# mengcaopku/DCNet

Hardware: AMD Instinct MI355X
Metric: clips/sec (T=8, 416x416, bs8) fwd+bwd (higher is better)
Workload: dtype f32; 1 GPU; T=8 416x416 bs8/GPU L=20 fp32, 64 img/GPU/step as pairs, fwd+5 losses+bwd+RMSprop; arith=f16x2-split MFMA, fp32 accumulate, parallelism=dp1, ranks_seen=1, reducer=none, step=hipGraph replay (fwd+losses+bwd+RMSprop), sampler=mt

## Files before the change

dcnet_amd/csrc/conv1.hip:

```cpp
#include "igemm.h"
#include "prof.h"

namespace {

typedef _Float16 f16x8_t __attribute__((ext_vector_type(8)));
typedef _Float16 f16x4_t __attribute__((ext_vector_type(4)));
typedef __attribute__((address_space(3))) void lds_void;

constexpr unsigned C1_OOB = 0x80000000u;

__device__ __forceinline__ float c1_pow2_scale(unsigned amax_bits) {
  const int be = (int)((amax_bits >> 23) & 0xFF);
  if (be == 0 || be == 255) return 1.f;
  int e = 14 - (be - 126);
  e = e > 100 ? 100 : (e < -100 ? -100 : e);
  return __uint_as_float((unsigned)(e + 127) << 23);
}

#ifndef C1_OCC
#define C1_OCC 4
#endif
template <int SA, int SB, int NI, int MI>
__global__ __launch_bounds__(256, (NI == 4 && MI == 1) ? C1_OCC : 2) void conv1_kernel(const IgemmParams p) {
  constexpr int BM = 128 * MI, BN = 32 * NI;
  constexpr int ASTAGE = BM * 64, BPLANE = BN * 32, BSTAGE = 2 * BPLANE;
  constexpr int AP = 4 * MI;
  constexpr int NLD = AP > NI ? AP : NI;
  extern __shared__ __attribute__((aligned(1024))) unsigned char smem1[];
  const int tid = threadIdx.x, lane = tid & 63;
  const int wave = __builtin_amdgcn_readfirstlane(tid >> 6);
  const int gn = p.Co / BN;
  const int lin = xcd_remap(blockIdx.x, gridDim.x);
  const int bm = lin / gn, bn = lin - bm * gn;
  const int M = p.M, m0 = bm * BM;
  const int cpt = p.Ci >> 4;
  const int kiters = p.ntaps * cpt;
  const int hsws = p.Hs * p.Ws;
  const bool plain = p.ntaps == 1 && p.dense_out && p.isy == 1 && p.isx == 1 && p.tap_dy[0] == 0 && p.tap_dx[0] == 0 &&
                     p.Ws == p.Wi && p.Hs == p.Hi;

  const float sa = c1_pow2_scale(amax_read(p.amax_a)), sb = p.b_scale[0];

  const int n0 = m0 / hsws;
  const long long img = (long long)p.Hi * p.Wi * p.ldi;
  const float* a_base = p.in + (long long)n0 * img;
  const long long a_bytes = ((long long)(p.N - n0) * img - p.ldi + p.Ci) * 4;
  const __amdgpu_buffer_rsrc_t a_rs = __builtin_amdgcn_make_buffer_rsrc((void*)a_base, 0, a_bytes > 0x7FFFFFF0LL ? 0x7FFFFFF0 : (int)a_bytes, 0x00020000);
  const __amdgpu_buffer_rsrc_t b_rs = __builtin_amdgcn_make_buffer_rsrc((void*)p.wt, 0, (int)((long long)p.Co * p.ldw * 4), 0x00020000);

  const bool loads_a = wave < 2;
  unsigned voff[NLD], msk[NLD];
#pragma unroll
  for (int e = 0; e < NLD; ++e) { voff[e] = C1_OOB; msk[e] = 0; }
  if (loads_a) {
#pragma unroll
    for (int e = 0; e < AP; ++e) {
      const int j = AP * (wave & 1) + e;
      const int row = 16 * j + (lane >> 2), cp = lane & 3, c = cp ^ ((row >> 2) & 3);
      const int m = m0 + row;
      if (m < M) {
        if (plain) { voff[e] = (unsigned)((m - n0 * hsws) * p.ldi * 4 + c * 16); msk[e] = 1u; }
        else {
          const int n = m / hsws, rem = m - n * hsws;
          const int i = rem / p.Ws, jx = rem - i * p.Ws;
          const int iy0 = i * p.isy, ix0 = jx * p.isx;
          voff[e] = (unsigned)((((n - n0) * p.Hi + iy0) * p.Wi + ix0) * p.ldi * 4 + c * 16);
          unsigned mk = 0;
          for (int t = 0; t < p.ntaps; ++t)
            if ((unsigned)(iy0 + p.tap_dy[t]) < (unsigned)p.Hi && (unsigned)(ix0 + p.tap_dx[t]) < (unsigned)p.Wi) mk |= 1u << t;
          msk[e] = mk;
        }
      }
    }
  } else {
#pragma unroll
    for (int e = 0; e < NI; ++e) {
      const int plane = wave & 1, rr = 32 * e + (lane >> 1), kh = (lane & 1) ^ ((rr >> 3) & 1);
      voff[e] = (unsigned)((bn * BN + rr) * p.ldw * 4 + (2 * kh + plane) * 16);
      msk[e] = 0xFFFFu;
    }
  }
  const __amdgpu_buffer_rsrc_t my_rs = loads_a ? a_rs : b_rs;
  const int my_dst = loads_a ? AP * (wave & 1) * 1024 : SA * ASTAGE + (wave & 1) * BPLANE;
  const int my_n = loads_a ? AP : NI;

  int k_tap = 0, k_c = 0, k_done = 0;
  auto issue = [&]() {
    const bool live = k_done < kiters;
    const unsigned bit = 1u << k_tap;
    int delta = 0; unsigned soff = 0;
    if (live) {
      if (loads_a) { delta = (p.tap_dy[k_tap] * p.Wi + p.tap_dx[k_tap]) * p.ldi * 4; soff = (unsigned)k_c * 64u; }
      else soff = (unsigned)(p.tap_w[k_tap] + k_c * 16) * 4u;
    }
    unsigned char* st = smem1 + (loads_a ? (k_done % SA) * ASTAGE : (k_done % SB) * BSTAGE) + my_dst;
#pragma unroll
    for (int e = 0; e < NLD; ++e)
      if (e < my_n)
        __builtin_amdgcn_raw_ptr_buffer_load_lds(my_rs, (lds_void*)(st + e * 1024), 16,
                                                 (int)((live && (msk[e] & bit)) ? voff[e] + (unsigned)delta : C1_OOB), (int)soff, 0, 0);
    ++k_done; ++k_c;
    if (k_c == cpt) { k_c = 0; ++k_tap; }
  };

  const int kh = lane >> 5;
  int a_rd0[MI], a_rd1[MI];
#pragma unroll
  for (int mi = 0; mi < MI; ++mi) {
    const int ar = (wave * MI + mi) * 32 + (lane & 31);
    a_rd0[mi] = ar * 64 + (((2 * kh) ^ ((ar >> 2) & 3)) << 4);
    a_rd1[mi] = ar * 64 + (((2 * kh + 1) ^ ((ar >> 2) & 3)) << 4);
  }
  int b_rd[NI];
#pragma unroll
  for (int ni = 0; ni < NI; ++ni) {
    const int row = ni * 32 + (lane & 31);
    b_rd[ni] = SA * ASTAGE + row * 32 + (((kh ^ (row >> 3)) & 1) << 4);
  }

  f32x16 acc[MI][NI];
#pragma unroll
  for (int mi = 0; mi < MI; ++mi)
#pragma unroll
    for (int ni = 0; ni < NI; ++ni)
#pragma unroll
      for (int r = 0; r < 16; ++r) acc[mi][ni][r] = 0.f;

  for (int s = 0; s < (loads_a ? SA : SB) - 1; ++s) issue();

  for (int it = 0; it < kiters; ++it) {
    if (loads_a) asm volatile("s_waitcnt vmcnt(%0)" :: "n"((SA - 2) * AP) : "memory");
    else asm volatile("s_waitcnt vmcnt(%0)" :: "n"((SB - 2) * NI) : "memory");
    __builtin_amdgcn_s_barrier();
    asm volatile("" ::: "memory");
    issue();
    const unsigned char* st = smem1 + (it % SA) * ASTAGE;
    const unsigned char* sb_ = smem1 + (it % SB) * BSTAGE;
    f16x8_t bh[NI], bl[NI];
#pragma unroll
    for (int ni = 0; ni < NI; ++ni) {
      bh[ni] = *reinterpret_cast<const f16x8_t*>(sb_ + b_rd[ni]);
      bl[ni] = *reinterpret_cast<const f16x8_t*>(sb_ + BPLANE + b_rd[ni]);
    }
    f16x8_t ah[MI], al[MI];
#pragma unroll
    for (int mi = 0; mi < MI; ++mi) {
      const f32x4 x0 = *reinterpret_cast<const f32x4*>(st + a_rd0[mi]), x1 = *reinterpret_cast<const f32x4*>(st + a_rd1[mi]);
      const f32x4 t0 = x0 * sa, t1 = x1 * sa;
#pragma unroll
      for (int e = 0; e < 4; ++e) { ah[mi][e] = (_Float16)t0[e]; ah[mi][4 + e] = (_Float16)t1[e]; }
#pragma unroll
      for (int e = 0; e < 4; ++e) { al[mi][e] = (_Float16)(t0[e] - (float)ah[mi][e]); al[mi][4 + e] = (_Float16)(t1[e] - (float)ah[mi][4 + e]); }
    }
#pragma unroll
    for (int mi = 0; mi < MI; ++mi)
#pragma unroll
      for (int ni = 0; ni < NI; ++ni) acc[mi][ni] = __builtin_amdgcn_mfma_f32_32x32x16_f16(al[mi], bh[ni], acc[mi][ni], 0, 0, 0);
#pragma unroll
    for (int mi = 0; mi < MI; ++mi)
#pragma unroll
      for (int ni = 0; ni < NI; ++ni) acc[mi][ni] = __builtin_amdgcn_mfma_f32_32x32x16_f16(ah[mi], bl[ni], acc[mi][ni], 0, 0, 0);
#pragma unroll
    for (int mi = 0; mi < MI; ++mi)
#pragma unroll
      for (int ni = 0; ni < NI; ++ni) acc[mi][ni] = __builtin_amdgcn_mfma_f32_32x32x16_f16(ah[mi], bh[ni], acc[mi][ni], 0, 0, 0);
  }
  asm volatile("s_waitcnt vmcnt(0)" ::: "memory");
  __syncthreads();

  const float dq = 1.f / (sa * sb);
#pragma unroll
  for (int mi = 0; mi < MI; ++mi)
#pragma unroll
    for (int ni = 0; ni < NI; ++ni) acc[mi][ni] *= dq;

  float* __restrict__ gout = p.out;
  auto out_pix = [&](int m) -> size_t {
    if (p.dense_out) return (size_t)m;
    const int n = m / hsws, rem = m - n * hsws;
    const int i = rem / p.Ws, jx = rem - i * p.Ws;
    return ((size_t)n * p.Ho + p.oy0 + i * p.osy) * p.Wo + p.ox0 + jx * p.osx;
  };
  if (p.accumulate) {
#pragma unroll
    for (int mi = 0; mi < MI; ++mi)
#pragma unroll
      for (int r = 0; r < 16; ++r) {
        const int m = m0 + (wave * MI + mi) * 32 + 4 * kh + (r & 3) + 8 * (r >> 2);
        if (m >= M) continue;
        const size_t pix = out_pix(m);
#pragma unroll
        for (int ni = 0; ni < NI; ++ni) acc[mi][ni][r] += gout[pix * p.ldo + bn * BN + ni * 32 + (lane & 31)];
      }
  }
  if (p.stats) {
    float* red = reinterpret_cast<float*>(smem1);
#pragma unroll
    for (int ni = 0; ni < NI; ++ni) {
      float s = 0.f, ss = 0.f;
      if (p.bt_y) {
        const int co = bn * BN + ni * 32 + (lane & 31);
        const float mu = p.bt_mean[co], is = p.bt_invstd[co], ga = p.bt_gamma ? p.bt_gamma[co] : 1.f, be = p.bt_beta ? p.bt_beta[co] : 0.f;
        const float* yb = p.bt_y + co;
        float yv[MI][16];
#pragma unroll
        for (int mi = 0; mi < MI; ++mi)
#pragma unroll
          for (int r = 0; r < 16; ++r) {
            const int m = m0 + (wave * MI + mi) * 32 + 4 * kh + (r & 3) + 8 * (r >> 2);
            yv[mi][r] = yb[(size_t)(m < M ? m : M - 1) * p.Co];
          }
#pragma unroll
        for (int mi = 0; mi < MI; ++mi)
#pragma unroll
          for (int r = 0; r < 16; ++r) {
            const int m = m0 + (wave * MI + mi) * 32 + 4 * kh + (r & 3) + 8 * (r >> 2);
            const float xh = (yv[mi][r] - mu) * is;
            float g = acc[mi][ni][r];
            if (p.bt_act == DCN_ACT_LEAKY) g = (ga * xh + be <= 0.f) ? g * p.bt_slope : g;
            g = m < M ? g : 0.f;
            s += g; ss += g * xh;
          }
      } else {
#pragma unroll
        for (int mi = 0; mi < MI; ++mi)
#pragma unroll
          for (int r = 0; r < 16; ++r) { const float v = acc[mi][ni][r]; s += v; ss = __builtin_fmaf(v, v, ss); }
      }
      s += __shfl_xor(s, 32); ss += __shfl_xor(ss, 32);
      if (lane < 32) {
        red[(0 * 4 + wave) * BN + ni * 32 + lane] = s;
        red[(1 * 4 + wave) * BN + ni * 32 + lane] = ss;
      }
    }
    __syncthreads();
    for (int idx = tid; idx < 2 * BN; idx += 256) {
      const int which = idx / BN, col = idx - which * BN;
      float t = 0.f;
#pragma unroll
      for (int w = 0; w < 4; ++w) t += red[(which * 4 + w) * BN + col];
      p.stats[((size_t)bm * 2 + which) * p.Co + bn * BN + col] = t;
    }
  }
  float sc[NI], sh[NI];
#pragma unroll
  for (int ni = 0; ni < NI; ++ni) {
    const int co = bn * BN + ni * 32 + (lane & 31);
    sc[ni] = p.scale ? p.scale[co] : 1.f;
    sh[ni] = p.shift ? p.shift[co] : 0.f;
  }
  float vmax = 0.f;
#pragma unroll
  for (int mi = 0; mi < MI; ++mi)
#pragma unroll
    for (int r = 0; r < 16; ++r) {
      const int m = m0 + (wave * MI + mi) * 32 + 4 * kh + (r & 3) + 8 * (r >> 2);
      if (m >= M) continue;
      const size_t pix = out_pix(m);
#pragma unroll
      for (int ni = 0; ni < NI; ++ni) {
        const int co = bn * BN + ni * 32 + (lane & 31);
        float v = acc[mi][ni][r] * sc[ni] + sh[ni];
        if (p.act == DCN_ACT_LEAKY) v = v > 0.f ? v : v * p.slope;
        if (p.residual) v += p.residual[pix * p.ldr + co];
        gout[pix * p.ldo + co] = v;
        vmax = fmaxf(vmax, fabsf(v));
      }
    }
  if (p.amax_out) {
    vmax = wave_max(vmax);
    if (lane == 0) amax_update(p.amax_out, vmax, blockIdx.x * 4 + wave);
  }
}

typedef __bf16 bf16x8_t __attribute__((ext_vector_type(8)));

template <bool O32> struct OutT { typedef __bf16 type; };
template <> struct OutT<true> { typedef float type; };

typedef int v8i_t __attribute__((ext_vector_type(8)));
typedef int v4i_t __attribute__((ext_vector_type(4)));
template <int I> struct IC1 { static constexpr int value = I; };
template <int N, int I = 0, typename F> __device__ __forceinline__ void static_for1(F&& f) {
  if constexpr (I < N) { f(IC1<I>{}); static_for1<N, I + 1>(f); }
}

template <int SA, int SB, int NI, int MI, bool O32, bool F8 = false>
__global__ __launch_bounds__(256, 2) void conv1b_kernel(const IgemmParams p) {
  typedef typename OutT<O32>::type out_t;
  constexpr int ESZ = F8 ? 1 : 2, KSTEP = 64 / ESZ;
  constexpr int BM = 128 * MI, BN = 32 * NI;
  constexpr int ASTAGE = BM * 64, BSTAGE = BN * 64;
  constexpr int AP = 4 * MI;
  constexpr int NLD = AP > NI ? AP : NI;
  extern __shared__ __attribute__((aligned(1024))) unsigned char smem1[];
  const int tid = threadIdx.x, lane = tid & 63;
  const int wave = __builtin_amdgcn_readfirstlane(tid >> 6);
  const int gn = p.Co / BN;
  const int lin = xcd_remap(blockIdx.x, gridDim.x);
  const int bm = lin / gn, bn = lin - bm * gn;
  const int M = p.M, m0 = bm * BM;
  const int cpt = p.Ci / KSTEP;
  const int kiters = p.ntaps * cpt;
  const int hsws = p.Hs * p.Ws;
  const bool plain = p.ntaps == 1 && p.dense_out && p.isy == 1 && p.isx == 1 && p.tap_dy[0] == 0 && p.tap_dx[0] == 0 &&
                     p.Ws == p.Wi && p.Hs == p.Hi;

  const int n0 = m0 / hsws;
  const long long img = (long long)p.Hi * p.Wi * p.ldi;
  const char* a_base = reinterpret_cast<const char*>(p.in) + (long long)n0 * img * ESZ;
  const long long a_bytes = ((long long)(p.N - n0) * img - p.ldi + p.Ci) * ESZ;
  const __amdgpu_buffer_rsrc_t a_rs = __builtin_amdgcn_make_buffer_rsrc((void*)a_base, 0, a_bytes > 0x7FFFFFF0LL ? 0x7FFFFFF0 : (int)a_bytes, 0x00020000);
  const __amdgpu_buffer_rsrc_t b_rs = __builtin_amdgcn_make_buffer_rsrc((void*)p.wt, 0, (int)((long long)p.Co * p.ldw * ESZ), 0x00020000);

  const bool loads_a = wave < 2;
  unsigned voff[NLD], msk[NLD];
#pragma unroll
  for (int e = 0; e < NLD; ++e) { voff[e] = C1_OOB; msk[e] = 0; }
  if (loads_a) {
#pragma unroll
    for (int e = 0; e < AP; ++e) {
      const int j = AP * (wave & 1) + e;
      const int row = 16 * j + (lane >> 2), cp = lane & 3, c = cp ^ ((row >> 2) & 3);
      const int m = m0 + row;
      if (m < M) {
        if (plain) { voff[e] = (unsigned)((m - n0 * hsws) * p.ldi * ESZ + c * 16); msk[e] = 1u; }
        else {
          const int n = m / hsws, rem = m - n * hsws;
          const int i = rem / p.Ws, jx = rem - i * p.Ws;
          const int iy0 = i * p.isy, ix0 = jx * p.isx;
          voff[e] = (unsigned)((((n - n0) * p.Hi + iy0) * p.Wi + ix0) * p.ldi * ESZ + c * 16);
          unsigned mk = 0;
          for (int t = 0; t < p.ntaps; ++t)
            if ((unsigned)(iy0 + p.tap_dy[t]) < (unsigned)p.Hi && (unsigned)(ix0 + p.tap_dx[t]) < (unsigned)p.Wi) mk |= 1u << t;
          msk[e] = mk;
        }
      }
    }
  } else {
#pragma unroll
    for (int e = 0; e < NI; ++e) {
      const int j = NI * (wave & 1) + e;
      const int row = 16 * j + (lane >> 2), cp = lane & 3, c = cp ^ ((row >> 2) & 3);
      voff[e] = (unsigned)((bn * BN + row) * p.ldw * ESZ + c * 16);
      msk[e] = 0xFFFFu;
    }
  }
  const __amdgpu_buffer_rsrc_t my_rs = loads_a ? a_rs : b_rs;
  const int my_dst = loads_a ? AP * (wave & 1) * 1024 : SA * ASTAGE + NI * (wave & 1) * 1024;
  const int my_n = loads_a ? AP : NI;

  int k_tap = 0, k_c = 0, k_done = 0;
  auto issue = [&]() {
    const bool live = k_done < kiters;
    const unsigned bit = 1u << k_tap;
    int delta = 0; unsigned soff = 0;
    if (live) {
      if (loads_a) { delta = (p.tap_dy[k_tap] * p.Wi + p.tap_dx[k_tap]) * p.ldi * ESZ; soff = (unsigned)k_c * 64u; }
      else soff = (unsigned)(p.tap_w[k_tap] + k_c * KSTEP) * (unsigned)ESZ;
    }
    unsigned char* st = smem1 + (loads_a ? (k_done % SA) * ASTAGE : (k_done % SB) * BSTAGE) + my_dst;
#pragma unroll
    for (int e = 0; e < NLD; ++e)
      if (e < my_n)
        __builtin_amdgcn_raw_ptr_buffer_load_lds(my_rs, (lds_void*)(st + e * 1024), 16,
                                                 (int)((live && (msk[e] & bit)) ? voff[e] + (unsigned)delta : C1_OOB), (int)soff, 0, 0);
    ++k_done; ++k_c;
    if (k_c == cpt) { k_c = 0; ++k_tap; }
  };

  const int kh = lane >> 5;
  int a_rd[MI][2], b_rd[NI][2];
#pragma unroll
  for (int kb = 0; kb < 2; ++kb) {
#pragma unroll
    for (int mi = 0; mi < MI; ++mi) {
      const int ar = (wave * MI + mi) * 32 + (lane & 31);
      a_rd[mi][kb] = ar * 64 + ((((F8 ? 2 * kh + kb : 2 * kb + kh)) ^ ((ar >> 2) & 3)) << 4);
    }
#pragma unroll
    for (int ni = 0; ni < NI; ++ni) {
      const int row = ni * 32 + (lane & 31);
      b_rd[ni][kb] = SA * ASTAGE + row * 64 + ((((F8 ? 2 * kh + kb : 2 * kb + kh)) ^ ((row >> 2) & 3)) << 4);
    }
  }
  unsigned sa_pk[MI][3], sb_pk[2];
  if constexpr (F8) {
    const unsigned char* as8 = reinterpret_cast<const unsigned char*>(p.a_scale8);
    const unsigned char* bs8 = reinterpret_cast<const unsigned char*>(p.b_scale8);
#pragma unroll
    for (int mi = 0; mi < MI; ++mi) {
      const int m = m0 + (wave * MI + mi) * 32 + (lane & 31);
      long long pix = -1; int iy0 = 0, ix0 = 0;
      if (m < M) {
        if (plain) pix = m;
        else {
          const int n = m / hsws, rem = m - n * hsws;
          const int i = rem / p.Ws, jx = rem - i * p.Ws;
          iy0 = i * p.isy; ix0 = jx * p.isx;
          pix = ((long long)n * p.Hi + iy0) * p.Wi + ix0;
        }
      }
#pragma unroll
      for (int w = 0; w < 3; ++w) {
        unsigned pk = 0;
#pragma unroll
        for (int b = 0; b < 4; ++b) {
          const int t = 4 * w + b;
          unsigned v = 127u;
          if (t < p.ntaps && pix >= 0 && (plain || ((unsigned)(iy0 + p.tap_dy[t]) < (unsigned)p.Hi && (unsigned)(ix0 + p.tap_dx[t]) < (unsigned)p.Wi)))
            v = as8[pix + p.tap_dy[t] * p.Wi + p.tap_dx[t]];
          pk |= v << (8 * b);
        }
        sa_pk[mi][w] = pk;
      }
    }
#pragma unroll
    for (int w = 0; w < 2; ++w) {
      unsigned pk = 0;
#pragma unroll
      for (int b = 0; b < 4; ++b) { const int ni = 4 * w + b; if (ni < NI) pk |= (unsigned)bs8[bn * BN + ni * 32 + (lane & 31)] << (8 * b); }
      sb_pk[w] = pk;
    }
#pragma unroll
    for (int mi = 0; mi < MI; ++mi)
#pragma unroll
      for (int w = 0; w < 3; ++w) asm volatile("" : "+v"(sa_pk[mi][w]));
    asm volatile("" : "+v"(sb_pk[0]), "+v"(sb_pk[1]));
  }
  int c_tap = 0, c_kc = 0;

  f32x16 acc[MI][NI];
#pragma unroll
  for (int mi = 0; mi < MI; ++mi)
#pragma unroll
    for (int ni = 0; ni < NI; ++ni)
#pragma unroll
      for (int r = 0; r < 16; ++r) acc[mi][ni][r] = 0.f;

  for (int s = 0; s < (loads_a ? SA : SB) - 1; ++s) issue();

  for (int it = 0; it < kiters; ++it) {
    if (loads_a) asm volatile("s_waitcnt vmcnt(%0)" :: "n"((SA - 2) * AP) : "memory");
    else asm volatile("s_waitcnt vmcnt(%0)" :: "n"((SB - 2) * NI) : "memory");
    __builtin_amdgcn_s_barrier();
    asm volatile("" ::: "memory");
    issue();
    const unsigned char* st = smem1 + (it % SA) * ASTAGE;
    const unsigned char* sb_ = smem1 + (it % SB) * BSTAGE;
    bf16x8_t af[MI][2], bf[NI][2];
#pragma unroll
    for (int kb = 0; kb < 2; ++kb) {
#pragma unroll
      for (int ni = 0; ni < NI; ++ni) bf[ni][kb] = *reinterpret_cast<const bf16x8_t*>(sb_ + b_rd[ni][kb]);
#pragma unroll
      for (int mi = 0; mi < MI; ++mi) af[mi][kb] = *reinterpret_cast<const bf16x8_t*>(st + a_rd[mi][kb]);
    }
    if constexpr (F8) {
      unsigned sa_now[MI];
#pragma unroll
      for (int mi = 0; mi < MI; ++mi) {
        const unsigned w = c_tap < 4 ? sa_pk[mi][0] : (c_tap < 8 ? sa_pk[mi][1] : sa_pk[mi][2]);
        sa_now[mi] = (w >> (8 * (c_tap & 3))) & 0xFFu;
      }
      if (++c_kc == cpt) { c_kc = 0; ++c_tap; }
#pragma unroll
      for (int mi = 0; mi < MI; ++mi) {
        const v4i_t a0 = __builtin_bit_cast(v4i_t, af[mi][0]), a1 = __builtin_bit_cast(v4i_t, af[mi][1]);
        const v8i_t a8 = {a0[0], a0[1], a0[2], a0[3], a1[0], a1[1], a1[2], a1[3]};
        static_for1<NI>([&](auto nic) {
          constexpr int ni = decltype(nic)::value;
          const v4i_t b0 = __builtin_bit_cast(v4i_t, bf[ni][0]), b1 = __builtin_bit_cast(v4i_t, bf[ni][1]);
          const v8i_t b8 = {b0[0], b0[1], b0[2], b0[3], b1[0], b1[1], b1[2], b1[3]};
          acc[mi][ni] = __builtin_amdgcn_mfma_scale_f32_32x32x64_f8f6f4(a8, b8, acc[mi][ni], 0, 0, 0, (int)sa_now[mi], ni & 3, (int)sb_pk[ni >> 2]);
        });
      }
    } else {
#pragma unroll
      for (int kb = 0; kb < 2; ++kb)
#pragma unroll
        for (int mi = 0; mi < MI; ++mi)
#pragma unroll
          for (int ni = 0; ni < NI; ++ni) acc[mi][ni] = __builtin_amdgcn_mfma_f32_32x32x16_bf16(af[mi][kb], bf[ni][kb], acc[mi][ni], 0, 0, 0);
    }
  }
  asm volatile("s_waitcnt vmcnt(0)" ::: "memory");
  __syncthreads();

  out_t* __restrict__ gout = reinterpret_cast<out_t*>(p.out);
  auto out_pix = [&](int m) -> size_t {
    if (p.dense_out) return (size_t)m;
    const int n = m / hsws, rem = m - n * hsws;
    const int i = rem / p.Ws, jx = rem - i * p.Ws;
    return ((size_t)n * p.Ho + p.oy0 + i * p.osy) * p.Wo + p.ox0 + jx * p.osx;
  };
  if (p.accumulate) {
#pragma unroll
    for (int mi = 0; mi < MI; ++mi)
#pragma unroll
      for (int r = 0; r < 16; ++r) {
        const int m = m0 + (wave * MI + mi) * 32 + 4 * kh + (r & 3) + 8 * (r >> 2);
        if (m >= M) continue;
        const size_t pix = out_pix(m);
#pragma unroll
        for (int ni = 0; ni < NI; ++ni) acc[mi][ni][r] += (float)gout[pix * p.ldo + bn * BN + ni * 32 + (lane & 31)];
      }
  }
  if (p.stats) {
    float* red = reinterpret_cast<float*>(smem1);
#pragma unroll
    for (int ni = 0; ni < NI; ++ni) {
      float s = 0.f, ss = 0.f;
      if (p.bt_y) {
        const int co = bn * BN + ni * 32 + (lane & 31);
        const float mu = p.bt_mean[co], is = p.bt_invstd[co], ga = p.bt_gamma ? p.bt_gamma[co] : 1.f, be = p.bt_beta ? p.bt_beta[co] : 0.f;
        const __bf16* yb = reinterpret_cast<const __bf16*>(p.bt_y) + co;
        float yv[MI][16];
#pragma unroll
        for (int mi = 0; mi < MI; ++mi)
#pragma unroll
          for (int r = 0; r < 16; ++r) {
            const int m = m0 + (wave * MI + mi) * 32 + 4 * kh + (r & 3) + 8 * (r >> 2);
            yv[mi][r] = (float)yb[(size_t)(m < M ? m : M - 1) * p.Co];
          }
#pragma unroll
        for (int mi = 0; mi < MI; ++mi)
#pragma unroll
          for (int r = 0; r < 16; ++r) {
            const int m = m0 + (wave * MI + mi) * 32 + 4 * kh + (r & 3) + 8 * (r >> 2);
            const float xh = (yv[mi][r] - mu) * is;
            float g = O32 ? acc[mi][ni][r] : (float)(__bf16)acc[mi][ni][r];
            if (p.bt_act == DCN_ACT_LEAKY) g = (ga * xh + be <= 0.f) ? g * p.bt_slope : g;
            g = m < M ? g : 0.f;
            s += g; ss += g * xh;
          }
      } else {
#pragma unroll
        for (int mi = 0; mi < MI; ++mi)
#pragma unroll
          for (int r = 0; r < 16; ++r) {
            const float v = O32 ? acc[mi][ni][r] : (float)(__bf16)acc[mi][ni][r];
            s += v; ss = __builtin_fmaf(v, v, ss);
          }
      }
      s += __shfl_xor(s, 32); ss += __shfl_xor(ss, 32);
      if (lane < 32) {
        red[(0 * 4 + wave) * BN + ni * 32 + lane] = s;
        red[(1 * 4 + wave) * BN + ni * 32 + lane] = ss;
      }
    }
    __syncthreads();
    for (int idx = tid; idx < 2 * BN; idx += 256) {
      const int which = idx / BN, col = idx - which * BN;
      float t = 0.f;
#pragma unroll
      for (int w = 0; w < 4; ++w) t += red[(which * 4 + w) * BN + col];
      p.stats[((size_t)bm * 2 + which) * p.Co + bn * BN + col] = t;
    }
  }
  float sc[NI], sh[NI];
#pragma unroll
  for (int ni = 0; ni < NI; ++ni) {
    const int co = bn * BN + ni * 32 + (lane & 31);
    sc[ni] = p.scale ? p.scale[co] : 1.f;
    sh[ni] = p.shift ? p.shift[co] : 0.f;
  }
  const __bf16* res16 = reinterpret_cast<const __bf16*>(p.residual);
#pragma unroll
  for (int mi = 0; mi < MI; ++mi)
#pragma unroll
    for (int r = 0; r < 16; ++r) {
      const int m = m0 + (wave * MI + mi) * 32 + 4 * kh + (r & 3) + 8 * (r >> 2);
      if (m >= M) continue;
      const size_t pix = out_pix(m);
#pragma unroll
      for (int ni = 0; ni < NI; ++ni) {
        const int co = bn * BN + ni * 32 + (lane & 31);
        float v = acc[mi][ni][r] * sc[ni] + sh[ni];
        if (p.act == DCN_ACT_LEAKY) v = v > 0.f ? v : v * p.slope;
        if (res16) v += (float)res16[pix * p.ldr + co];
        gout[pix * p.ldo + co] = (out_t)v;
      }
    }
}

DCN_KNOB(g_conv1, "1x1dma", 1, "conv1.hip: NT launches with a pre-split bank on the LDS-DMA kernel (0 = implicit-GEMM tiles of igemm.hip; 2 = 1x1 launches only)");
DCN_KNOB(g_conv1_stages, "1stages", 32, "conv1.hip: ring depths of the 128 x 128 tile, 10 * SA + SB (32 | 33 | 42 | 44 | 63)");

template <int SA, int SB, int NI, int MI>
int launch1(const IgemmParams& p, hipStream_t stream) {
  constexpr int BM = 128 * MI, BN = 32 * NI;
  static DcnPerDeviceFlag attr_once;
  const size_t lds = (size_t)SA * BM * 64 + (size_t)SB * 2 * BN * 32;
  if (attr_once.first()) {
    (void)hipFuncSetAttribute(reinterpret_cast<const void*>(&conv1_kernel<SA, SB, NI, MI>), hipFuncAttributeMaxDynamicSharedMemorySize, (int)lds);
  }
  const int gm = cdiv(p.M, BM), gn = p.Co / BN;
  const double k_alg = (double)p.ntaps * p.Ci;
  const double alg_bytes = 4.0 * ((double)p.N * p.Hi * p.Wi * p.Ci + (double)p.Co * k_alg + (double)p.M * p.Co * epilogue_reads(p));
  const int pid = prof_begin(35, 2.0 * (double)p.M * p.Co * k_alg, stream, alg_bytes);
  hipLaunchKernelGGL((conv1_kernel<SA, SB, NI, MI>), dim3(gm * gn), dim3(256), lds, stream, p);
  prof_end(pid, stream);
  DCN_CHECK_LAUNCH("conv1");
  return DCN_OK;
}

template <int NI, int MI>
int launch1_ring(const IgemmParams& p, hipStream_t stream) {
  if constexpr (NI == 4 && MI == 1) {
    switch (g_conv1_stages) {
      case 33: return launch1<3, 3, NI, MI>(p, stream);
      case 42: return launch1<4, 2, NI, MI>(p, stream);
      case 44: return launch1<4, 4, NI, MI>(p, stream);
      case 63: return launch1<6, 3, NI, MI>(p, stream);
      default: break;
    }
  }
  return launch1<3, 2, NI, MI>(p, stream);
}

DCN_KNOB(g_conv1_wide, "1wide", 1024, "conv1.hip: 128 x 256 tiles from that many workgroups on (0 = off)");

int conv1_shape(const IgemmParams& p, int gran) {
  int ni = p.Co % 128 == 0 ? 4 : (p.Co % 64 == 0 ? 2 : (p.Co % 32 == 0 ? 1 : 0));
  if (!ni) return 0;
  if (g_conv1_wide && p.Co % 256 == 0 && (!p.stats || gran == 128) && (long long)cdiv(p.M, 128) * (p.Co / 256) >= g_conv1_wide) return 18;
  int mi;
  if (p.stats) { mi = gran == 128 ? 1 : (gran == 256 ? 2 : 0); }
  else mi = ni == 4 ? 1 : 2;
  if (!mi || mi * ni > 4 || (mi == 1 && ni == 1)) return 0;
  return mi * 10 + ni;
}

DCN_KNOB(g_conv1b_wide, "bwide", 1024, "conv1.hip: bf16- / fp8-storage 128 x 256 tiles from that many workgroups on (0 = off)");
int conv1b_shape(int M, int Co) {
  if (Co % 32 != 0) return 0;
  if (g_conv1b_wide && Co % 256 == 0 && (long long)cdiv(M, 128) * (Co / 256) >= g_conv1b_wide) return 18;
  if (Co % 128 == 0) return 14;
  if (Co % 64 == 0) return 12;
  return 21;
}

template <int NI, int MI, bool O32, bool F8 = false>
int launch1b(const IgemmParams& p, hipStream_t stream) {
  constexpr int SA = 3, SB = 2;
  constexpr int BM = 128 * MI, BN = 32 * NI;
  static DcnPerDeviceFlag attr_once;
  const size_t lds = (size_t)SA * BM * 64 + (size_t)SB * BN * 64;
  if (attr_once.first()) {
    (void)hipFuncSetAttribute(reinterpret_cast<const void*>(&conv1b_kernel<SA, SB, NI, MI, O32, F8>), hipFuncAttributeMaxDynamicSharedMemorySize, (int)lds);
  }
  const int gm = cdiv(p.M, BM), gn = p.Co / BN;
  const double k_alg = (double)p.ntaps * p.Ci;
  const double alg_bytes = (F8 ? 1.0 : 2.0) * ((double)p.N * p.Hi * p.Wi * p.Ci + (double)p.Co * k_alg) +
                           ((O32 ? 4.0 : 2.0) * (1.0 + (p.accumulate ? 1.0 : 0.0) + (p.residual ? 1.0 : 0.0)) + (p.bt_y ? 2.0 : 0.0)) * (double)p.M * p.Co;
  const int pid = prof_begin(F8 ? 48 : 41, 2.0 * (double)p.M * p.Co * k_alg, stream, alg_bytes);
  hipLaunchKernelGGL((conv1b_kernel<SA, SB, NI, MI, O32, F8>), dim3(gm * gn), dim3(256), lds, stream, p);
  prof_end(pid, stream);
  DCN_CHECK_LAUNCH("conv1b");
  return DCN_OK;
}

}

bool conv1_will_take(long long rows, int Co, int ntaps, int Ci) {
  if (!g_conv1 || rows < 1024 || Co % 64 != 0 || Ci % 16 != 0 || Ci < 32 || ntaps < 1 || ntaps > 16) return false;
  if (g_conv1 == 2 && ntaps != 1) return false;
  return true;
}

int conv1_tile_of(long long rows, int Co, int ntaps, int Ci, int stats, int gran, int storage16) {
  if (storage16) return conv1b_shape((int)rows, Co);
  if (!conv1_will_take(rows, Co, ntaps, Ci)) return 0;
  static float one_word;
  IgemmParams p{};
  p.M = (int)rows; p.Co = Co; p.ntaps = ntaps; p.Ci = Ci; p.stats = stats ? &one_word : nullptr;
  return conv1_shape(p, gran);
}

bool conv1_applicable(const IgemmParams& p, int precision, int gran) {
  if (!g_conv1 || precision != 4 || !p.b_scale || !p.amax_a || p.wt16 || p.f8 || p.c4 || p.bmode != 0 || p.batch > 1 || p.row_scale || p.ncls)
    return false;
  if (!conv1_will_take(p.M, p.Co, p.ntaps, p.Ci)) return false;
  if (p.ntaps > 1 && p.isy == 1 && p.osy == 1) return false;
  if ((long long)p.M != (long long)p.N * p.Hs * p.Ws) return false;
  if (p.Hs * p.Ws < 1 || (256 / (p.Hs * p.Ws) + 2) * (long long)p.Hi * p.Wi * p.ldi * 4 >= 0x7FFFFFF0LL || (long long)p.Co * p.ldw * 4 >= 0x7FFFFFF0LL) return false;
  return conv1_shape(p, gran) != 0;
}

int conv1_launch(const IgemmParams& p, int gran, hipStream_t stream) {
  switch (conv1_shape(p, gran)) {
    case 18: return launch1_ring<8, 1>(p, stream);
    case 14: return launch1_ring<4, 1>(p, stream);
    case 12: return launch1_ring<2, 1>(p, stream);
    case 22: return launch1_ring<2, 2>(p, stream);
    case 21: return launch1_ring<1, 2>(p, stream);
    default: dcn_set_error("conv1: no tile for this launch"); return DCN_ERR_ARG;
  }
}

int conv1b_grid_m(int M, int Co, int ntaps, int s1_w) {
  if (ntaps == 9 && s1_w > 0) { const int bm3 = conv3b_bm(M, Co, s1_w); if (bm3) return cdiv(M, bm3); }
  if (conv2b_takes(M, Co, ntaps)) return cdiv(M, 256);
  const int sh = conv1b_shape(M, Co);
  return sh ? cdiv(M, 128 * (sh / 10)) : 0;
}

int conv1b_launch(const IgemmParams& p, int out_f32, hipStream_t stream) {
  if (p.Ci % 32 != 0 || p.c4 || p.bmode != 0 || p.batch > 1 || p.row_scale || p.ncls || p.ntaps < 1 || p.ntaps > 16 ||
      (long long)p.M != (long long)p.N * p.Hs * p.Ws) {
    dcn_set_error("conv1b: launch form not supported on bf16 storage (Ci=%d taps=%d)", p.Ci, p.ntaps); return DCN_ERR_ARG;
  }
  if (p.Hs * p.Ws < 1 || (256 / (p.Hs * p.Ws) + 2) * (long long)p.Hi * p.Wi * p.ldi * 2 >= 0x7FFFFFF0LL || (long long)p.Co * p.ldw * 2 >= 0x7FFFFFF0LL) {
    dcn_set_error("conv1b: tensor beyond the 2 GiB buffer window"); return DCN_ERR_ARG;
  }
  if (conv3b_takes(p)) return conv3b_launch(p, out_f32, stream);
  if (p.stats && p.ntaps == 9 && p.isy == 1 && p.isx == 1 && p.osy == 1 && p.osx == 1 && p.dense_out && conv3b_bm(p.M, p.Co, p.Wi) != 0) {
    dcn_set_error("conv1b: the strip kernel sized this launch's BatchNorm partials but cannot take it (tensor beyond its 2 GiB window)");
    return DCN_ERR_ARG;
  }
  if (conv2b_takes(p.M, p.Co, p.ntaps)) return conv2b_launch(p, out_f32, stream);
  switch (conv1b_shape(p.M, p.Co)) {
    case 18: return out_f32 ? launch1b<8, 1, true>(p, stream) : launch1b<8, 1, false>(p, stream);
    case 14: return out_f32 ? launch1b<4, 1, true>(p, stream) : launch1b<4, 1, false>(p, stream);
    case 12: return out_f32 ? launch1b<2, 1, true>(p, stream) : launch1b<2, 1, false>(p, stream);
    case 21: return out_f32 ? launch1b<1, 2, true>(p, stream) : launch1b<1, 2, false>(p, stream);
    default: dcn_set_error("conv1b: Co=%d is not a multiple of 32", p.Co); return DCN_ERR_ARG;
  }
}

int conv1q_grid_m(int M, int Co) {
  const int sh = conv1b_shape(M, Co);
  return sh ? cdiv(M, 128 * (sh / 10)) : 0;
}

int conv1q_launch(const IgemmParams& p, int out_f32, hipStream_t stream) {
  if (p.Ci % 64 != 0 || !p.a_scale8 || !p.b_scale8 || p.c4 || p.bmode != 0 || p.batch > 1 || p.row_scale || p.ncls || p.ntaps < 1 || p.ntaps > 12 ||
      (long long)p.M != (long long)p.N * p.Hs * p.Ws) {
    dcn_set_error("conv1q: launch form not supported on fp8 storage (Ci=%d taps=%d)", p.Ci, p.ntaps); return DCN_ERR_ARG;
  }
  if (p.Hs * p.Ws < 1 || (256 / (p.Hs * p.Ws) + 2) * (long long)p.Hi * p.Wi * p.ldi >= 0x7FFFFFF0LL || (long long)p.Co * p.ldw >= 0x7FFFFFF0LL) {
    dcn_set_error("conv1q: tensor beyond the 2 GiB buffer window"); return DCN_ERR_ARG;
  }
  switch (conv1b_shape(p.M, p.Co)) {
    case 18: return out_f32 ? launch1b<8, 1, true, true>(p, stream) : launch1b<8, 1, false, true>(p, stream);
    case 14: return out_f32 ? launch1b<4, 1, true, true>(p, stream) : launch1b<4, 1, false, true>(p, stream);
    case 12: return out_f32 ? launch1b<2, 1, true, true>(p, stream) : launch1b<2, 1, false, true>(p, stream);
    case 21: return out_f32 ? launch1b<1, 2, true, true>(p, stream) : launch1b<1, 2, false, true>(p, stream);
    default: dcn_set_error("conv1q: Co=%d is not a multiple of 32", p.Co); return DCN_ERR_ARG;
  }
}
```

Baseline: 87.90 clips/s.

## Permute conv1 filter columns per lane to vectorize epilogue loads and stores

```diff
diff --git a/dcnet_amd/csrc/conv1.hip b/dcnet_amd/csrc/conv1.hip
--- a/dcnet_amd/csrc/conv1.hip
+++ b/dcnet_amd/csrc/conv1.hip
@@ -20,8 +20,12 @@
 #ifndef C1_OCC
 #define C1_OCC 4
 #endif
-template <int SA, int SB, int NI, int MI>
+#ifndef C1_PERM
+#define C1_PERM 1
+#endif
+template <int SA, int SB, int NI, int MI, bool PERM>
 __global__ __launch_bounds__(256, (NI == 4 && MI == 1) ? C1_OCC : 2) void conv1_kernel(const IgemmParams p) {
+  static_assert(!PERM || NI >= 2, "a permuted tile needs two filters per lane to form a vector");
   constexpr int BM = 128 * MI, BN = 32 * NI;
   constexpr int ASTAGE = BM * 64, BPLANE = BN * 32, BSTAGE = 2 * BPLANE;
   constexpr int AP = 4 * MI;
@@ -76,7 +80,8 @@
 #pragma unroll
     for (int e = 0; e < NI; ++e) {
       const int plane = wave & 1, rr = 32 * e + (lane >> 1), kh = (lane & 1) ^ ((rr >> 3) & 1);
-      voff[e] = (unsigned)((bn * BN + rr) * p.ldw * 4 + (2 * kh + plane) * 16);
+      const int f = PERM ? NI * (lane >> 1) + e : rr;
+      voff[e] = (unsigned)((bn * BN + f) * p.ldw * 4 + (2 * kh + plane) * 16);
       msk[e] = 0xFFFFu;
     }
   }
@@ -181,6 +186,161 @@
     const int i = rem / p.Ws, jx = rem - i * p.Ws;
     return ((size_t)n * p.Ho + p.oy0 + i * p.osy) * p.Wo + p.ox0 + jx * p.osx;
   };
+  if constexpr (PERM) {
+    constexpr int NV = NI >= 4 ? 4 : 2, NC = NI / NV;
+    typedef float vec_t __attribute__((ext_vector_type(NV)));
+    const int co0 = bn * BN + NI * (lane & 31);
+    auto row_of = [&](int mi, int r) { return m0 + (wave * MI + mi) * 32 + 4 * kh + (r & 3) + 8 * (r >> 2); };
+    auto ldv = [&](const float* q, float (&dst)[NI]) {
+#pragma unroll
+      for (int c = 0; c < NC; ++c) {
+        const vec_t t = *reinterpret_cast<const vec_t*>(q + co0 + c * NV);
+#pragma unroll
+        for (int j = 0; j < NV; ++j) dst[c * NV + j] = t[j];
+      }
+    };
+    if (p.accumulate) {
+#pragma unroll
+      for (int mi = 0; mi < MI; ++mi)
+#pragma unroll
+        for (int r = 0; r < 16; ++r) {
+          const int m = row_of(mi, r);
+          if (m >= M) continue;
+          const float* q = gout + out_pix(m) * p.ldo + co0;
+#pragma unroll
+          for (int c = 0; c < NC; ++c) {
+            const vec_t t = *reinterpret_cast<const vec_t*>(q + c * NV);
+#pragma unroll
+            for (int j = 0; j < NV; ++j) acc[mi][c * NV + j][r] += t[j];
+          }
+        }
+    }
+    if (p.stats) {
+      float* red = reinterpret_cast<float*>(smem1);
+      float s[NI], ss[NI];
+#pragma unroll
+      for (int ni = 0; ni < NI; ++ni) { s[ni] = 0.f; ss[ni] = 0.f; }
+      if (p.bt_y) {
+        constexpr int GR = 2, TG = 16 * MI / GR;
+        auto ldc = [&](const float* q, int c, float fill, float (&dst)[NV]) {
+          vec_t t = fill;
+          if (q) t = *reinterpret_cast<const vec_t*>(q + co0 + c * NV);
+#pragma unroll
+          for (int j = 0; j < NV; ++j) dst[j] = t[j];
+        };
+#pragma unroll
+        for (int c = 0; c < NC; ++c) {
+          float mu[NV], is[NV], ga[NV], be[NV];
+          ldc(p.bt_mean, c, 0.f, mu); ldc(p.bt_invstd, c, 0.f, is); ldc(p.bt_gamma, c, 1.f, ga); ldc(p.bt_beta, c, 0.f, be);
+          const float* yb = p.bt_y + (size_t)m0 * p.Co;
+          int lim = M - 1 - m0;
+          asm("" : "+s"(lim));
+          vec_t yv[2][GR];
+          auto yload = [&](int t, vec_t (&dst)[GR]) {
+#pragma unroll
+            for (int q = 0; q < GR; ++q) {
+              const int u = t * GR + q, m = row_of(u >> 4, u & 15);
+              const int rl = m - m0;
+              dst[q] = *reinterpret_cast<const vec_t*>(yb + (unsigned)((rl < lim ? rl : lim) * p.Co + co0 + c * NV));
+            }
+          };
+          yload(0, yv[0]);
+#pragma unroll
+          for (int t = 0; t < TG; ++t) {
+            if (t + 1 < TG) yload(t + 1, yv[(t + 1) & 1]);
+#pragma unroll
+            for (int q = 0; q < GR; ++q) {
+              const int u = t * GR + q, mi = u >> 4, r = u & 15;
+              const int m = row_of(mi, r);
+#pragma unroll
+              for (int j = 0; j < NV; ++j) {
+                const int ni = c * NV + j;
+                float xh = (yv[t & 1][q][j] - mu[j]) * is[j];
+                asm("" : "+v"(xh));
+                float g = acc[mi][ni][r];
+                if (p.bt_act == DCN_ACT_LEAKY) g = (ga[j] * xh + be[j] <= 0.f) ? g * p.bt_slope : g;
+                g = m < M ? g : 0.f;
+                {
+#pragma clang fp contract(off)
+                  const float gx = g * xh;
+                  s[ni] += g; ss[ni] += gx;
+                }
+              }
+            }
+            __builtin_amdgcn_sched_barrier(0);
+          }
+        }
+      } else {
+#pragma unroll
+        for (int ni = 0; ni < NI; ++ni)
+#pragma unroll
+          for (int mi = 0; mi < MI; ++mi)
+#pragma unroll
+            for (int r = 0; r < 16; ++r) { const float v = acc[mi][ni][r]; s[ni] += v; ss[ni] = __builtin_fmaf(v, v, ss[ni]); }
+      }
+#pragma unroll
+      for (int ni = 0; ni < NI; ++ni) { s[ni] += __shfl_xor(s[ni], 32); ss[ni] += __shfl_xor(ss[ni], 32); }
+      if (lane < 32) {
+#pragma unroll
+        for (int c = 0; c < NC; ++c) {
+          vec_t t0, t1;
+#pragma unroll
+          for (int j = 0; j < NV; ++j) { t0[j] = s[c * NV + j]; t1[j] = ss[c * NV + j]; }
+          *reinterpret_cast<vec_t*>(red + (0 * 4 + wave) * BN + NI * lane + c * NV) = t0;
+          *reinterpret_cast<vec_t*>(red + (1 * 4 + wave) * BN + NI * lane + c * NV) = t1;
+        }
+      }
+      __syncthreads();
+      for (int idx = tid; idx < 2 * BN; idx += 256) {
+        const int which = idx / BN, col = idx - which * BN;
+        float t = 0.f;
+#pragma unroll
+        for (int w = 0; w < 4; ++w) t += red[(which * 4 + w) * BN + col];
+        p.stats[((size_t)bm * 2 + which) * p.Co + bn * BN + col] = t;
+      }
+    }
+    float sc[NI], sh[NI];
+    if (p.scale) ldv(p.scale, sc);
+    else {
+#pragma unroll
+      for (int ni = 0; ni < NI; ++ni) sc[ni] = 1.f;
+    }
+    if (p.shift) ldv(p.shift, sh);
+    else {
+#pragma unroll
+      for (int ni = 0; ni < NI; ++ni) sh[ni] = 0.f;
+    }
+    float vmax = 0.f;
+#pragma unroll
+    for (int mi = 0; mi < MI; ++mi)
+#pragma unroll
+      for (int r = 0; r < 16; ++r) {
+        const int m = row_of(mi, r);
+        if (m >= M) continue;
+        const size_t pix = out_pix(m);
+#pragma unroll
+        for (int c = 0; c < NC; ++c) {
+          vec_t res = {};
+          if (p.residual) res = *reinterpret_cast<const vec_t*>(p.residual + pix * p.ldr + co0 + c * NV);
+          vec_t o;
+#pragma unroll
+          for (int j = 0; j < NV; ++j) {
+            const int ni = c * NV + j;
+            float v = acc[mi][ni][r] * sc[ni] + sh[ni];
+            if (p.act == DCN_ACT_LEAKY) v = v > 0.f ? v : v * p.slope;
+            if (p.residual) v += res[j];
+            o[j] = v;
+            vmax = fmaxf(vmax, fabsf(v));
+          }
+          *reinterpret_cast<vec_t*>(gout + pix * p.ldo + co0 + c * NV) = o;
+        }
+      }
+    if (p.amax_out) {
+      vmax = wave_max(vmax);
+      if (lane == 0) amax_update(p.amax_out, vmax, blockIdx.x * 4 + wave);
+    }
+    return;
+  }
   if (p.accumulate) {
 #pragma unroll
     for (int mi = 0; mi < MI; ++mi)
@@ -587,36 +747,55 @@
 DCN_KNOB(g_conv1, "1x1dma", 1, "conv1.hip: NT launches with a pre-split bank on the LDS-DMA kernel (0 = implicit-GEMM tiles of igemm.hip; 2 = 1x1 launches only)");
 DCN_KNOB(g_conv1_stages, "1stages", 32, "conv1.hip: ring depths of the 128 x 128 tile, 10 * SA + SB (32 | 33 | 42 | 44 | 63)");
 
-template <int SA, int SB, int NI, int MI>
+bool conv1_perm_ok(const IgemmParams& p, int ni) {
+  if (ni < 2) return false;
+  const uintptr_t mask = ni >= 4 ? 15 : 7;
+  auto al = [mask](const void* q) { return (reinterpret_cast<uintptr_t>(q) & mask) == 0; };
+  if (p.Co % 4 != 0 || p.ldo % 4 != 0 || p.ldr % 4 != 0) return false;
+  return al(p.out) && al(p.residual) && al(p.bt_y) && al(p.scale) && al(p.shift) && al(p.bt_mean) && al(p.bt_invstd) && al(p.bt_gamma) &&
+         al(p.bt_beta);
+}
+
+template <int SA, int SB, int NI, int MI, bool PERM>
 int launch1(const IgemmParams& p, hipStream_t stream) {
   constexpr int BM = 128 * MI, BN = 32 * NI;
   static DcnPerDeviceFlag attr_once;
   const size_t lds = (size_t)SA * BM * 64 + (size_t)SB * 2 * BN * 32;
   if (attr_once.first()) {
-    (void)hipFuncSetAttribute(reinterpret_cast<const void*>(&conv1_kernel<SA, SB, NI, MI>), hipFuncAttributeMaxDynamicSharedMemorySize, (int)lds);
+    (void)hipFuncSetAttribute(reinterpret_cast<const void*>(&conv1_kernel<SA, SB, NI, MI, PERM>), hipFuncAttributeMaxDynamicSharedMemorySize, (int)lds);
   }
   const int gm = cdiv(p.M, BM), gn = p.Co / BN;
   const double k_alg = (double)p.ntaps * p.Ci;
   const double alg_bytes = 4.0 * ((double)p.N * p.Hi * p.Wi * p.Ci + (double)p.Co * k_alg + (double)p.M * p.Co * epilogue_reads(p));
   const int pid = prof_begin(35, 2.0 * (double)p.M * p.Co * k_alg, stream, alg_bytes);
-  hipLaunchKernelGGL((conv1_kernel<SA, SB, NI, MI>), dim3(gm * gn), dim3(256), lds, stream, p);
+  hipLaunchKernelGGL((conv1_kernel<SA, SB, NI, MI, PERM>), dim3(gm * gn), dim3(256), lds, stream, p);
   prof_end(pid, stream);
   DCN_CHECK_LAUNCH("conv1");
   return DCN_OK;
 }
 
-template <int NI, int MI>
+template <int NI, int MI, bool PERM>
 int launch1_ring(const IgemmParams& p, hipStream_t stream) {
   if constexpr (NI == 4 && MI == 1) {
     switch (g_conv1_stages) {
-      case 33: return launch1<3, 3, NI, MI>(p, stream);
-      case 42: return launch1<4, 2, NI, MI>(p, stream);
-      case 44: return launch1<4, 4, NI, MI>(p, stream);
-      case 63: return launch1<6, 3, NI, MI>(p, stream);
+      case 33: return launch1<3, 3, NI, MI, PERM>(p, stream);
+      case 42: return launch1<4, 2, NI, MI, PERM>(p, stream);
+      case 44: return launch1<4, 4, NI, MI, PERM>(p, stream);
+      case 63: return launch1<6, 3, NI, MI, PERM>(p, stream);
       default: break;
     }
   }
-  return launch1<3, 2, NI, MI>(p, stream);
+  return launch1<3, 2, NI, MI, PERM>(p, stream);
+}
+
+template <int NI, int MI>
+int launch1_perm(const IgemmParams& p, hipStream_t stream) {
+#if C1_PERM
+  if constexpr (NI >= 2) {
+    if (conv1_perm_ok(p, NI)) return launch1_ring<NI, MI, true>(p, stream);
+  }
+#endif
+  return launch1_ring<NI, MI, false>(p, stream);
 }
 
 DCN_KNOB(g_conv1_wide, "1wide", 1024, "conv1.hip: 128 x 256 tiles from that many workgroups on (0 = off)");
@@ -690,11 +869,11 @@
 
 int conv1_launch(const IgemmParams& p, int gran, hipStream_t stream) {
   switch (conv1_shape(p, gran)) {
-    case 18: return launch1_ring<8, 1>(p, stream);
-    case 14: return launch1_ring<4, 1>(p, stream);
-    case 12: return launch1_ring<2, 1>(p, stream);
-    case 22: return launch1_ring<2, 2>(p, stream);
-    case 21: return launch1_ring<1, 2>(p, stream);
+    case 18: return launch1_perm<8, 1>(p, stream);
+    case 14: return launch1_perm<4, 1>(p, stream);
+    case 12: return launch1_perm<2, 1>(p, stream);
+    case 22: return launch1_perm<2, 2>(p, stream);
+    case 21: return launch1_perm<1, 2>(p, stream);
     default: dcn_set_error("conv1: no tile for this launch"); return DCN_ERR_ARG;
   }
 }
```

Measured after the change: 87.88 clips/s. No clear change (-0.0%).

## Permute conv1 weight columns so each lane owns contiguous output channels for vector epilogue

Applied to the files above, without the earlier changes.

```diff
diff --git a/dcnet_amd/csrc/conv1.hip b/dcnet_amd/csrc/conv1.hip
--- a/dcnet_amd/csrc/conv1.hip
+++ b/dcnet_amd/csrc/conv1.hip
@@ -17,11 +17,49 @@
   return __uint_as_float((unsigned)(e + 127) << 23);
 }
 
+#ifndef C1_EPI
+#define C1_EPI 1
+#endif
+#ifndef C1_ABL
+#define C1_ABL 0
+#endif
+typedef float f32x2_t __attribute__((ext_vector_type(2)));
+template <int I> struct IC1 { static constexpr int value = I; };
+
+template <int NI, bool VEC> __device__ __forceinline__ void c1_ld(const float* q, float (&v)[NI]) {
+  if constexpr (VEC && NI % 4 == 0) {
+#pragma unroll
+    for (int j = 0; j < NI; j += 4) {
+      const f32x4 t = *reinterpret_cast<const f32x4*>(q + j);
+      v[j] = t[0]; v[j + 1] = t[1]; v[j + 2] = t[2]; v[j + 3] = t[3];
+    }
+  } else if constexpr (VEC && NI == 2) {
+    const f32x2_t t = *reinterpret_cast<const f32x2_t*>(q);
+    v[0] = t[0]; v[1] = t[1];
+  } else {
+#pragma unroll
+    for (int j = 0; j < NI; ++j) v[j] = q[j];
+  }
+}
+template <int NI, bool VEC> __device__ __forceinline__ void c1_st(float* q, const float (&v)[NI]) {
+  if constexpr (VEC && NI % 4 == 0) {
+#pragma unroll
+    for (int j = 0; j < NI; j += 4) { const f32x4 t = {v[j], v[j + 1], v[j + 2], v[j + 3]}; *reinterpret_cast<f32x4*>(q + j) = t; }
+  } else if constexpr (VEC && NI == 2) {
+    const f32x2_t t = {v[0], v[1]};
+    *reinterpret_cast<f32x2_t*>(q) = t;
+  } else {
+#pragma unroll
+    for (int j = 0; j < NI; ++j) q[j] = v[j];
+  }
+}
+
 #ifndef C1_OCC
 #define C1_OCC 4
 #endif
-template <int SA, int SB, int NI, int MI>
+template <int SA, int SB, int NI, int MI, bool VEC = false>
 __global__ __launch_bounds__(256, (NI == 4 && MI == 1) ? C1_OCC : 2) void conv1_kernel(const IgemmParams p) {
+  constexpr bool EPI = C1_EPI && !(NI == 2 && MI == 1);
   constexpr int BM = 128 * MI, BN = 32 * NI;
   constexpr int ASTAGE = BM * 64, BPLANE = BN * 32, BSTAGE = 2 * BPLANE;
   constexpr int AP = 4 * MI;
@@ -76,7 +114,8 @@
 #pragma unroll
     for (int e = 0; e < NI; ++e) {
       const int plane = wave & 1, rr = 32 * e + (lane >> 1), kh = (lane & 1) ^ ((rr >> 3) & 1);
-      voff[e] = (unsigned)((bn * BN + rr) * p.ldw * 4 + (2 * kh + plane) * 16);
+      const int f = EPI ? NI * (lane >> 1) + e : rr;
+      voff[e] = (unsigned)((bn * BN + f) * p.ldw * 4 + (2 * kh + plane) * 16);
       msk[e] = 0xFFFFu;
     }
   }
@@ -175,12 +214,130 @@
     for (int ni = 0; ni < NI; ++ni) acc[mi][ni] *= dq;
 
   float* __restrict__ gout = p.out;
-  auto out_pix = [&](int m) -> size_t {
+  auto out_pix = [&](int m) __attribute__((always_inline)) -> size_t {
     if (p.dense_out) return (size_t)m;
     const int n = m / hsws, rem = m - n * hsws;
     const int i = rem / p.Ws, jx = rem - i * p.Ws;
     return ((size_t)n * p.Ho + p.oy0 + i * p.osy) * p.Wo + p.ox0 + jx * p.osx;
   };
+  if constexpr (EPI) {
+  const auto e_accumulate = p.accumulate; const auto e_ldo = p.ldo; const auto e_stats = p.stats; const auto e_bt_y = p.bt_y;
+  const auto e_bt_mean = p.bt_mean; const auto e_bt_invstd = p.bt_invstd; const auto e_bt_gamma = p.bt_gamma; const auto e_bt_beta = p.bt_beta;
+  const auto e_Co = p.Co; const auto e_bt_act = p.bt_act; const auto e_bt_slope = p.bt_slope; const auto e_scale = p.scale;
+  const auto e_shift = p.shift; const auto e_residual = p.residual; const auto e_ldr = p.ldr; const auto e_act = p.act; const auto e_slope = p.slope;
+  const auto e_amax_out = p.amax_out; const auto e_dense_out = p.dense_out; const auto e_Ws = p.Ws; const auto e_Ho = p.Ho; const auto e_oy0 = p.oy0;
+  const auto e_osy = p.osy; const auto e_Wo = p.Wo; const auto e_ox0 = p.ox0; const auto e_osx = p.osx;
+  auto out_pix1 = [&](int m) __attribute__((always_inline)) -> size_t {
+    if (e_dense_out) return (size_t)m;
+    const int n = m / hsws, rem = m - n * hsws;
+    const int i = rem / e_Ws, jx = rem - i * e_Ws;
+    return ((size_t)n * e_Ho + e_oy0 + i * e_osy) * e_Wo + e_ox0 + jx * e_osx;
+  };
+  {
+    const int cl = bn * BN + NI * (lane & 31);
+    auto row_of = [&](int mi, int r) __attribute__((always_inline)) { return m0 + (wave * MI + mi) * 32 + 4 * kh + (r & 3) + 8 * (r >> 2); };
+    if (e_accumulate) {
+#pragma unroll
+      for (int mi = 0; mi < MI; ++mi)
+#pragma unroll
+        for (int r = 0; r < 16; ++r) {
+          const int m = row_of(mi, r);
+          if (m >= M) continue;
+          float t[NI];
+          c1_ld<NI, VEC>(gout + out_pix1(m) * e_ldo + cl, t);
+#pragma unroll
+          for (int ni = 0; ni < NI; ++ni) acc[mi][ni][r] += t[ni];
+        }
+    }
+    if (e_stats) {
+      float* red = reinterpret_cast<float*>(smem1);
+      float s[NI], ss[NI];
+#pragma unroll
+      for (int ni = 0; ni < NI; ++ni) { s[ni] = 0.f; ss[ni] = 0.f; }
+      if (e_bt_y) {
+        float mu[NI], is[NI], ga[NI], be[NI];
+        c1_ld<NI, VEC>(e_bt_mean + cl, mu); c1_ld<NI, VEC>(e_bt_invstd + cl, is);
+#pragma unroll
+        for (int ni = 0; ni < NI; ++ni) { ga[ni] = 1.f; be[ni] = 0.f; }
+        if (e_bt_gamma) c1_ld<NI, VEC>(e_bt_gamma + cl, ga);
+        if (e_bt_beta) c1_ld<NI, VEC>(e_bt_beta + cl, be);
+        const float* yb = e_bt_y + cl;
+#pragma unroll
+        for (int mi = 0; mi < MI; ++mi)
+#pragma unroll
+          for (int r = 0; r < 16; ++r) {
+            if (row_of(mi, r) >= M) continue;
+            float yv[NI];
+            c1_ld<NI, VEC>(yb + (size_t)row_of(mi, r) * e_Co, yv);
+#pragma unroll
+            for (int ni = 0; ni < NI; ++ni) {
+              float xh = (yv[ni] - mu[ni]) * is[ni];
+              float gr = acc[mi][ni][r];
+              asm("" : "+v"(xh), "+v"(gr));
+              if (e_bt_act == DCN_ACT_LEAKY) gr = (ga[ni] * xh + be[ni] <= 0.f) ? gr * e_bt_slope : gr;
+              s[ni] += gr; ss[ni] += gr * xh;
+            }
+          }
+      } else {
+#pragma unroll
+        for (int ni = 0; ni < NI; ++ni)
+#pragma unroll
+          for (int mi = 0; mi < MI; ++mi)
+#pragma unroll
+            for (int r = 0; r < 16; ++r) { const float v = acc[mi][ni][r]; s[ni] += v; ss[ni] = __builtin_fmaf(v, v, ss[ni]); }
+      }
+#pragma unroll
+      for (int ni = 0; ni < NI; ++ni) { s[ni] += __shfl_xor(s[ni], 32); ss[ni] += __shfl_xor(ss[ni], 32); }
+      if (lane < 32) {
+#pragma unroll
+        for (int ni = 0; ni < NI; ++ni) {
+          red[(0 * 4 + wave) * BN + NI * lane + ni] = s[ni];
+          red[(1 * 4 + wave) * BN + NI * lane + ni] = ss[ni];
+        }
+      }
+      __syncthreads();
+      for (int idx = tid; idx < 2 * BN; idx += 256) {
+        const int which = idx / BN, col = idx - which * BN;
+        float t = 0.f;
+#pragma unroll
+        for (int w = 0; w < 4; ++w) t += red[(which * 4 + w) * BN + col];
+        e_stats[((size_t)bm * 2 + which) * e_Co + bn * BN + col] = t;
+      }
+    }
+    float sc[NI], sh[NI];
+#pragma unroll
+    for (int ni = 0; ni < NI; ++ni) { sc[ni] = 1.f; sh[ni] = 0.f; }
+    if (e_scale) c1_ld<NI, VEC>(e_scale + cl, sc);
+    if (e_shift) c1_ld<NI, VEC>(e_shift + cl, sh);
+    float vmax = 0.f;
+#pragma unroll
+    for (int mi = 0; mi < MI; ++mi)
+#pragma unroll
+      for (int r = 0; r < 16; ++r) {
+        const int m = row_of(mi, r);
+        if (m >= M) continue;
+        const size_t pix = out_pix1(m);
+        float v[NI], rs[NI];
+        if (e_residual) c1_ld<NI, VEC>(e_residual + pix * e_ldr + cl, rs);
+#pragma unroll
+        for (int ni = 0; ni < NI; ++ni) {
+          float a = acc[mi][ni][r];
+          asm("" : "+v"(a));
+          v[ni] = a * sc[ni] + sh[ni];
+          if (e_act == DCN_ACT_LEAKY) v[ni] = v[ni] > 0.f ? v[ni] : v[ni] * e_slope;
+          if (e_residual) v[ni] += rs[ni];
+          vmax = fmaxf(vmax, fabsf(v[ni]));
+        }
+#if !C1_ABL
+        c1_st<NI, VEC>(gout + pix * e_ldo + cl, v);
+#endif
+      }
+    if (e_amax_out) {
+      vmax = wave_max(vmax);
+      if (lane == 0) amax_update(e_amax_out, vmax, blockIdx.x * 4 + wave);
+    }
+  }
+  } else {
   if (p.accumulate) {
 #pragma unroll
     for (int mi = 0; mi < MI; ++mi)
@@ -263,7 +420,9 @@
         float v = acc[mi][ni][r] * sc[ni] + sh[ni];
         if (p.act == DCN_ACT_LEAKY) v = v > 0.f ? v : v * p.slope;
         if (p.residual) v += p.residual[pix * p.ldr + co];
+#if !C1_ABL
         gout[pix * p.ldo + co] = v;
+#endif
         vmax = fmaxf(vmax, fabsf(v));
       }
     }
@@ -271,6 +430,7 @@
     vmax = wave_max(vmax);
     if (lane == 0) amax_update(p.amax_out, vmax, blockIdx.x * 4 + wave);
   }
+  }
 }
 
 typedef __bf16 bf16x8_t __attribute__((ext_vector_type(8)));
@@ -280,7 +440,6 @@
 
 typedef int v8i_t __attribute__((ext_vector_type(8)));
 typedef int v4i_t __attribute__((ext_vector_type(4)));
-template <int I> struct IC1 { static constexpr int value = I; };
 template <int N, int I = 0, typename F> __device__ __forceinline__ void static_for1(F&& f) {
   if constexpr (I < N) { f(IC1<I>{}); static_for1<N, I + 1>(f); }
 }
@@ -587,22 +746,32 @@
 DCN_KNOB(g_conv1, "1x1dma", 1, "conv1.hip: NT launches with a pre-split bank on the LDS-DMA kernel (0 = implicit-GEMM tiles of igemm.hip; 2 = 1x1 launches only)");
 DCN_KNOB(g_conv1_stages, "1stages", 32, "conv1.hip: ring depths of the 128 x 128 tile, 10 * SA + SB (32 | 33 | 42 | 44 | 63)");
 
-template <int SA, int SB, int NI, int MI>
-int launch1(const IgemmParams& p, hipStream_t stream) {
+template <int SA, int SB, int NI, int MI, bool VEC>
+int launch1v(const IgemmParams& p, hipStream_t stream) {
   constexpr int BM = 128 * MI, BN = 32 * NI;
   static DcnPerDeviceFlag attr_once;
   const size_t lds = (size_t)SA * BM * 64 + (size_t)SB * 2 * BN * 32;
   if (attr_once.first()) {
-    (void)hipFuncSetAttribute(reinterpret_cast<const void*>(&conv1_kernel<SA, SB, NI, MI>), hipFuncAttributeMaxDynamicSharedMemorySize, (int)lds);
+    (void)hipFuncSetAttribute(reinterpret_cast<const void*>(&conv1_kernel<SA, SB, NI, MI, VEC>), hipFuncAttributeMaxDynamicSharedMemorySize, (int)lds);
   }
   const int gm = cdiv(p.M, BM), gn = p.Co / BN;
   const double k_alg = (double)p.ntaps * p.Ci;
   const double alg_bytes = 4.0 * ((double)p.N * p.Hi * p.Wi * p.Ci + (double)p.Co * k_alg + (double)p.M * p.Co * epilogue_reads(p));
   const int pid = prof_begin(35, 2.0 * (double)p.M * p.Co * k_alg, stream, alg_bytes);
-  hipLaunchKernelGGL((conv1_kernel<SA, SB, NI, MI>), dim3(gm * gn), dim3(256), lds, stream, p);
+  hipLaunchKernelGGL((conv1_kernel<SA, SB, NI, MI, VEC>), dim3(gm * gn), dim3(256), lds, stream, p);
   prof_end(pid, stream);
   DCN_CHECK_LAUNCH("conv1");
   return DCN_OK;
+}
+
+template <int SA, int SB, int NI, int MI>
+int launch1(const IgemmParams& p, hipStream_t stream) {
+#if C1_EPI
+  const uintptr_t ptr_bits = (uintptr_t)p.out | (uintptr_t)p.residual | (uintptr_t)p.bt_y | (uintptr_t)p.scale | (uintptr_t)p.shift |
+                             (uintptr_t)p.bt_mean | (uintptr_t)p.bt_invstd | (uintptr_t)p.bt_gamma | (uintptr_t)p.bt_beta;
+  if (NI > 1 && !(NI == 2 && MI == 1) && (ptr_bits & 15) == 0 && ((p.ldo | (p.residual ? p.ldr : 0) | p.Co) & 3) == 0) return launch1v<SA, SB, NI, MI, true>(p, stream);
+#endif
+  return launch1v<SA, SB, NI, MI, false>(p, stream);
 }
 
 template <int NI, int MI>
```

Result: no change. 87.79 clips/s before, 88.03 clips/s after (median of 6 runs) (+0.3%).
